# musevlt/origin

Hardware: AMD Instinct MI355X
Metric: voxels/s through DCT+PCA+GLR (ORIGIN hot path) (higher is better)
Workload: dtype f32+f16x2; 1 GPU; synthetic 3681x600x600 cube, Dico_FWHM_2_12 (20 profiles), PSF 25x25, 100x100 areas, dct_order 10, pfa 0.01, Noise_population 50, itermax 100; masked_border=0, glr_spectral_arithmetic=f16x2, tiles=1

## Files before the change

### origin_amd/csrc/common.h

```cpp
#pragma once
#include <hip/hip_runtime.h>

#include <algorithm>
#include <cstdarg>
#include <cstdio>
#include <cstring>
#include <mutex>
#include <vector>

#include "../../include/origin_hip.h"

enum OriginKernelId {
  K_DCT_FIT = 0,
  K_DCT_SUMS,
  K_DCT_STANDARDIZE,
  K_DCT_CONTINUUM,
  K_O2,
  K_PCA_SELECT,
  K_PCA_BMEAN,
  K_PCA_GATHER,
  K_PCA_PROJECT,
  K_PCA_GRAM,
  K_PCA_EIG,
  K_PCA_UVEC,
  K_PCA_DEFLATE_DOT,
  K_PCA_DEFLATE_UPDATE,
  K_PCA_FLUSH,
  K_GLR_SPATIAL,
  K_GLR_SPECTRAL,
  K_GLR_BORDER,
  K_GLR_TABLES,
  K_LOCAL_MAX,
  K_SMALL,
  K_PCA_TOTAL,
  K_LINES_GATHER,
  K_LINES_UVEC,
  K_LINES_PROJECT,
  K_LINES_LS,
  K_LINES_SELECT,
  K_MERGE_BIN,
  K_MERGE_COMP,
  K_MERGE_STAGE1,
  K_MERGE_RENUMBER,
  K_MERGE_STAGE2,
  K_STATS,
  K_COUNT
};

struct OriginProfEvent {
  hipEvent_t a, b;
  int id;
};

constexpr int ORIGIN_TIMER_SLOTS = 64;

struct GrowBuffer {
  void *p = nullptr;
  size_t bytes = 0;
};

struct ForkStream {
  hipStream_t stream = nullptr;
  hipEvent_t fork = nullptr, join = nullptr;
  bool pending = false;
};

struct AllocCache;

struct origin_ctx {
  int device = 0;
  hipStream_t stream = nullptr;
  hipEvent_t ev_start[ORIGIN_TIMER_SLOTS] = {};
  hipEvent_t ev_stop[ORIGIN_TIMER_SLOTS] = {};
  bool ev_made[ORIGIN_TIMER_SLOTS] = {};
  GrowBuffer scratch;
  int num_cu = 0;
  double *ctab = nullptr;
  int ctab_nz = 0, ctab_order = 0;
  int prof_level = 0;
  std::vector<OriginProfEvent> prof_pending;
  std::vector<hipEvent_t> prof_free;
  double prof_ms[K_COUNT] = {};
  long prof_n[K_COUNT] = {};
  void *pca_ws = nullptr;
  void (*pca_ws_free)(void *) = nullptr;
  ForkStream aux;
  GrowBuffer aux_scratch;
  ForkStream side;
  char *stage_buf[2] = {nullptr, nullptr};
  hipEvent_t stage_ev[2] = {nullptr, nullptr};
  bool stage_ready = false;
  void (*pca_tail_hook)(void *user, int n_active, const int *areas) = nullptr;
  void *pca_tail_user = nullptr;
  int pca_tail_max = 0;
  AllocCache *alloc_cache = nullptr;
};

int origin_make_aux_stream(origin_ctx *ctx, hipStream_t *out);
int origin_make_side_stream(origin_ctx *ctx, hipStream_t *out);
int origin_fork_begin(origin_ctx *ctx, ForkStream &f, int (*create)(origin_ctx *, hipStream_t *));
int origin_fork_end(ForkStream &f);
int origin_fork_join(origin_ctx *ctx, ForkStream &f);
int origin_fork_wait(ForkStream &f);

int origin_prof_begin(origin_ctx *ctx, int id);
void origin_prof_end(origin_ctx *ctx, int entry);

struct ProfScope {
  origin_ctx *ctx;
  int entry;
  ProfScope(origin_ctx *c, int id, int level = 1) : ctx(c), entry(-1) {
    if (ctx->prof_level >= level) entry = origin_prof_begin(ctx, id);
  }
  void next(int id) {
    if (entry >= 0) {
      origin_prof_end(ctx, entry);
      entry = origin_prof_begin(ctx, id);
    }
  }
  ~ProfScope() {
    if (entry >= 0) origin_prof_end(ctx, entry);
  }
};

void origin_set_error(const char *fmt, ...);
int origin_grow(GrowBuffer &b, size_t bytes, hipStream_t sync, void **out);
static inline int origin_scratch(origin_ctx *ctx, size_t bytes, void **out) {
  return origin_grow(ctx->scratch, bytes, ctx->stream, out);
}

int origin_spatial_mfma_ok(int Ny, int Nx, int P);
int origin_spatial_mfma_launch(origin_ctx *ctx, int terms, const float *A, const float *W,
                               const float *taps, int Nz, int Ny, int Nx, int P, int accf,
                               float *out, int ry0 = 0, int nry = 0, int rx0 = 0, int nrx = 0);
long origin_spatial_mfma_count(int terms, int Nz, int Ny, int Nx, int P);

struct DevMem {
  origin_ctx *ctx;
  void *p = nullptr;
  explicit DevMem(origin_ctx *c) : ctx(c) {}
  int alloc(size_t bytes) { return origin_malloc(ctx, std::max(bytes, (size_t)256), &p); }
  ~DevMem() {
    if (p) (void)origin_free(ctx, p);
  }
};

struct Carver {
  size_t off = 0;
  char *base = nullptr;
  template <class T>
  T *take(size_t n) {
    T *r = base ? (T *)(base + off) : nullptr;
    off += (n * sizeof(T) + 255) & ~(size_t)255;
    return r;
  }
};

template <class Layout>
int carve_block(origin_ctx *ctx, DevMem &mem, Layout &&layout) {
  Carver c;
  layout(c);
  const int rc = mem.alloc(c.off);
  if (rc) return rc;
  c.off = 0, c.base = (char *)mem.p;
  layout(c);
  return ORIGIN_OK;
}

constexpr long IO_CHUNK_BYTES = 64l << 20;

struct IoStage {
  void *h[2] = {nullptr, nullptr};
  hipEvent_t ev[2] = {nullptr, nullptr};
  ~IoStage() {
    for (int i = 0; i < 2; ++i) {
      if (h[i]) (void)hipHostFree(h[i]);
      if (ev[i]) (void)hipEventDestroy(ev[i]);
    }
  }
};

template <class T>
int put(origin_ctx *ctx, T *d, const std::vector<T> &h) {
  return origin_h2d(ctx, d, h.data(), h.size() * sizeof(T));
}

#define ORIGIN_CHECK_ARG(cond, ...)       \
  do {                                    \
    if (!(cond)) {                        \
      origin_set_error(__VA_ARGS__);      \
      return ORIGIN_E_ARG;                \
    }                                     \
  } while (0)

#define ORIGIN_HIP(call)                                                              \
// ... 42 lines not shown
```

### origin_amd/csrc/ctx.hip

```cpp
#include <sys/mman.h>

#include <algorithm>
#include <cstdlib>
#include <map>
#include <unordered_map>

#include <functional>

#include <cstring>
#include "common.h"

void origin_host_pool_run(int n, const std::function<void(int)> &task);

static thread_local char g_err[1024] = "";

struct AllocCache {
  std::mutex mu;
  std::unordered_map<void *, size_t> live;
  std::multimap<size_t, void *> spare;
  size_t spare_bytes = 0, cap_bytes = 0;
};
constexpr size_t ALLOC_MIN = (size_t)1 << 20;

static size_t alloc_cache_spare(AllocCache *c) {
  std::lock_guard<std::mutex> lk(c->mu);
  return c->spare_bytes;
}

static void alloc_cache_release(origin_ctx *ctx, bool destroy) {
  AllocCache *c = ctx->alloc_cache;
  if (!c) return;
  {
    std::lock_guard<std::mutex> lk(c->mu);
    if (!c->spare.empty()) (void)hipStreamSynchronize(ctx->stream);
    for (auto &kv : c->spare) (void)hipFree(kv.second);
    c->spare.clear();
    c->spare_bytes = 0;
  }
  if (destroy) {
    delete c;
    ctx->alloc_cache = nullptr;
  }
}

__global__ __launch_bounds__(256) void copy_box_kernel(char *__restrict__ dst, long dpy, long dpz,
                                                       const char *__restrict__ src, long spy,
                                                       long spz, int ny, long rowbytes, int vec) {
  const int z = blockIdx.z;
  const int y = blockIdx.y;
  const long x = ((long)blockIdx.x * 256 + threadIdx.x) * vec;
  if (y >= ny || x >= rowbytes) return;
  const char *s = src + (long)z * spz + (long)y * spy + x;
  char *d = dst + (long)z * dpz + (long)y * dpy + x;
  if (vec == 16) {
    *reinterpret_cast<uint4 *>(d) = *reinterpret_cast<const uint4 *>(s);
  } else if (vec == 4) {
    *reinterpret_cast<unsigned *>(d) = *reinterpret_cast<const unsigned *>(s);
  } else {
    *d = *s;
  }
}

void origin_set_error(const char *fmt, ...) {
  va_list ap;
  va_start(ap, fmt);
  vsnprintf(g_err, sizeof(g_err), fmt, ap);
  va_end(ap);
}

int origin_grow(GrowBuffer &b, size_t bytes, hipStream_t sync, void **out) {
  if (bytes > b.bytes) {
    if (b.p) {
      if (sync) ORIGIN_HIP(hipStreamSynchronize(sync));
      ORIGIN_HIP(hipFree(b.p));
      b.p = nullptr;
      b.bytes = 0;
    }
    const size_t want = bytes + bytes / 4 + (1 << 20);
    ORIGIN_HIP(hipMalloc(&b.p, want));
    b.bytes = want;
  }
  *out = b.p;
  return ORIGIN_OK;
}

int origin_make_side_stream(origin_ctx *ctx, hipStream_t *out) {
  const char *e = getenv("ORIGIN_GLR_SIDE_RESERVE");
  const int ncu = ctx->num_cu > 0 ? std::min(ctx->num_cu, 256) : 256;
  int reserve = e ? atoi(e) : ncu / 8;
  reserve = std::max(0, std::min(reserve, ncu - 8));
  uint32_t mask[8] = {0, 0, 0, 0, 0, 0, 0, 0};
  for (int i = 0; i < ncu - reserve; ++i) mask[i >> 5] |= 1u << (i & 31);
  if (hipExtStreamCreateWithCUMask(out, 8, mask) != hipSuccess) {
    (void)hipGetLastError();
    return origin_make_aux_stream(ctx, out);
  }
  return ORIGIN_OK;
}

int origin_make_aux_stream(origin_ctx *, hipStream_t *out) {
  int lo = 0, hi = 0;
  ORIGIN_HIP(hipDeviceGetStreamPriorityRange(&lo, &hi));
  ORIGIN_HIP(hipStreamCreateWithPriority(out, hipStreamNonBlocking, lo));
  return ORIGIN_OK;
}

int origin_fork_begin(origin_ctx *ctx, ForkStream &f, int (*create)(origin_ctx *, hipStream_t *)) {
  if (!f.stream) {
    if (int rc = create(ctx, &f.stream)) return rc;
    ORIGIN_HIP(hipEventCreateWithFlags(&f.fork, hipEventDisableTiming));
    ORIGIN_HIP(hipEventCreateWithFlags(&f.join, hipEventDisableTiming));
  }
  ORIGIN_HIP(hipEventRecord(f.fork, ctx->stream));
  ORIGIN_HIP(hipStreamWaitEvent(f.stream, f.fork, 0));
  return ORIGIN_OK;
}

int origin_fork_end(ForkStream &f) {
  ORIGIN_HIP(hipEventRecord(f.join, f.stream));
  f.pending = true;
  return ORIGIN_OK;
}

int origin_fork_join(origin_ctx *ctx, ForkStream &f) {
  if (f.stream && f.pending) {
    ORIGIN_HIP(hipStreamWaitEvent(ctx->stream, f.join, 0));
    f.pending = false;
  }
  return ORIGIN_OK;
}

int origin_fork_wait(ForkStream &f) {
  if (f.stream && f.pending) {
    ORIGIN_HIP(hipStreamSynchronize(f.stream));
    f.pending = false;
  }
  return ORIGIN_OK;
}

static hipEvent_t prof_event(origin_ctx *ctx) {
  if (!ctx->prof_free.empty()) {
    hipEvent_t e = ctx->prof_free.back();
    ctx->prof_free.pop_back();
    return e;
  }
  hipEvent_t e = nullptr;
  (void)hipEventCreate(&e);
  return e;
}

static void prof_drain(origin_ctx *ctx) {
  for (auto &p : ctx->prof_pending) {
    float ms = 0.f;
    if (p.a && p.b && hipEventSynchronize(p.b) == hipSuccess &&
        hipEventElapsedTime(&ms, p.a, p.b) == hipSuccess) {
      ctx->prof_ms[p.id] += ms;
      ctx->prof_n[p.id] += 1;
    }
    if (p.a) ctx->prof_free.push_back(p.a);
    if (p.b) ctx->prof_free.push_back(p.b);
  }
  ctx->prof_pending.clear();
}

int origin_prof_begin(origin_ctx *ctx, int id) {
  OriginProfEvent p;
  p.a = prof_event(ctx);
  p.b = nullptr;
  p.id = id;
  if (p.a) (void)hipEventRecord(p.a, ctx->stream);
  ctx->prof_pending.push_back(p);
  return (int)ctx->prof_pending.size() - 1;
}

void origin_prof_end(origin_ctx *ctx, int entry) {
  if (entry < 0 || entry >= (int)ctx->prof_pending.size()) return;
  OriginProfEvent &p = ctx->prof_pending[entry];
  p.b = prof_event(ctx);
  if (p.b) (void)hipEventRecord(p.b, ctx->stream);
}

static const char *kKernelNames[K_COUNT] = {
    "dct_fit",         "dct_plane_sums",     "dct_standardize", "dct_continuum", "o2",
    "pca_select",      "pca_bmean",          "pca_gather",      "pca_project",   "pca_gram",
    "pca_eig",         "pca_uvec",
    "pca_deflate_dot", "pca_deflate_finish", "pca_flush", "glr_spatial",     "glr_spectral",  "glr_border", "glr_tables",
    "local_max",       "small",              "pca_total",
    "lines_gather",    "lines_uvec",         "lines_project",   "lines_ls",      "lines_select",
    "merge_bin",       "merge_components",   "merge_stage1",    "merge_renumber", "merge_stage2",
    "cube_moments"};

extern "C" {

int origin_prof_enable(origin_ctx *ctx, int on) {
  ORIGIN_USE(ctx);
  prof_drain(ctx);
  ctx->prof_level = on < 0 ? 0 : (on > 2 ? 2 : on);
  return ORIGIN_OK;
}

int origin_prof_reset(origin_ctx *ctx) {
  ORIGIN_USE(ctx);
  prof_drain(ctx);
  memset(ctx->prof_ms, 0, sizeof(ctx->prof_ms));
  memset(ctx->prof_n, 0, sizeof(ctx->prof_n));
  return ORIGIN_OK;
}

int origin_prof_count(void) { return K_COUNT; }

int origin_prof_get(origin_ctx *ctx, int id, const char **name, double *total_ms, long *launches) {
  ORIGIN_USE(ctx);
  ORIGIN_CHECK_ARG(id >= 0 && id < K_COUNT, "kernel id out of range");
  prof_drain(ctx);
  if (name) *name = kKernelNames[id];
  if (total_ms) *total_ms = ctx->prof_ms[id];
  if (launches) *launches = ctx->prof_n[id];
  return ORIGIN_OK;
}

const char *origin_last_error(void) { return g_err; }

int origin_abi_version(void) { return 1; }

int origin_device_count(int *count) {
  ORIGIN_CHECK_ARG(count, "count is null");
  int n = 0;
  hipError_t e = hipGetDeviceCount(&n);
  if (e != hipSuccess) {
    *count = 0;
    origin_set_error("hipGetDeviceCount: %s", hipGetErrorString(e));
    return ORIGIN_E_NODEVICE;
  }
  *count = n;
  return ORIGIN_OK;
}

int origin_ctx_create(int device, origin_ctx **out) {
  ORIGIN_CHECK_ARG(out, "out is null");
  int n = 0;
  if (hipGetDeviceCount(&n) != hipSuccess || n <= 0) {
    origin_set_error("no HIP device visible");
    return ORIGIN_E_NODEVICE;
  }
  ORIGIN_CHECK_ARG(device >= 0 && device < n, "device %d out of range [0,%d)", device, n);
  ORIGIN_HIP(hipSetDevice(device));
  origin_ctx *ctx = new origin_ctx();
  ctx->device = device;
  hipError_t e = hipStreamCreateWithFlags(&ctx->stream, hipStreamNonBlocking);
  if (e != hipSuccess) {
    delete ctx;
    origin_set_error("hipStreamCreate: %s", hipGetErrorString(e));
    return ORIGIN_E_HIP;
  }
  hipDeviceProp_t prop;
  if (hipGetDeviceProperties(&prop, device) == hipSuccess) ctx->num_cu = prop.multiProcessorCount;
  if (ctx->num_cu <= 0) ctx->num_cu = 256;
  ctx->alloc_cache = new AllocCache();
  const char *gb = getenv("ORIGIN_ALLOC_CACHE_GB");
  ctx->alloc_cache->cap_bytes = (size_t)((gb ? atof(gb) : 96.0) * 1e9);
  *out = ctx;
  return ORIGIN_OK;
}

int origin_ctx_destroy(origin_ctx *ctx) {
  if (!ctx) return ORIGIN_OK;
  hipSetDevice(ctx->device);
  hipStreamSynchronize(ctx->stream);
  for (int i = 0; i < ORIGIN_TIMER_SLOTS; ++i)
    if (ctx->ev_made[i]) {
      hipEventDestroy(ctx->ev_start[i]);
      hipEventDestroy(ctx->ev_stop[i]);
    }
  for (ForkStream *f : {&ctx->aux, &ctx->side})
    if (f->stream) {
      hipStreamSynchronize(f->stream);
      hipStreamDestroy(f->stream);
      hipEventDestroy(f->fork);
      hipEventDestroy(f->join);
    }
  if (ctx->stage_ready) {
    for (int b = 0; b < 2; ++b) {
      hipHostFree(ctx->stage_buf[b]);
      hipEventDestroy(ctx->stage_ev[b]);
    }
  }
  alloc_cache_release(ctx, true);
  if (ctx->aux_scratch.p) hipFree(ctx->aux_scratch.p);
  if (ctx->scratch.p) hipFree(ctx->scratch.p);
  if (ctx->ctab) hipFree(ctx->ctab);
  if (ctx->pca_ws && ctx->pca_ws_free) ctx->pca_ws_free(ctx->pca_ws);
  prof_drain(ctx);
  for (hipEvent_t e : ctx->prof_free) hipEventDestroy(e);
  hipStreamDestroy(ctx->stream);
  delete ctx;
  return ORIGIN_OK;
}

int origin_sync(origin_ctx *ctx) {
  ORIGIN_USE(ctx);
  if (int rc = origin_fork_wait(ctx->side)) return rc;
  ORIGIN_HIP(hipStreamSynchronize(ctx->stream));
  return origin_fork_wait(ctx->aux);
}

int origin_aux_join(origin_ctx *ctx) {
  ORIGIN_USE(ctx);
  return origin_fork_join(ctx, ctx->aux);
}

int origin_device_name(origin_ctx *ctx, char *buf, int buflen) {
  ORIGIN_USE(ctx);
  ORIGIN_CHECK_ARG(buf && buflen > 0, "bad buffer");
  hipDeviceProp_t prop;
  ORIGIN_HIP(hipGetDeviceProperties(&prop, ctx->device));
  snprintf(buf, buflen, "%s (%s, %d CUs)", prop.name, prop.gcnArchName, prop.multiProcessorCount);
  return ORIGIN_OK;
}

int origin_mem_info(origin_ctx *ctx, size_t *free_bytes, size_t *total_bytes) {
  ORIGIN_USE(ctx);
  size_t f = 0, t = 0;
  ORIGIN_HIP(hipMemGetInfo(&f, &t));
  if (free_bytes) *free_bytes = f + alloc_cache_spare(ctx->alloc_cache);
  if (total_bytes) *total_bytes = t;
  return ORIGIN_OK;
}

int origin_stream(origin_ctx *ctx, void **stream) {
  ORIGIN_USE(ctx);
  ORIGIN_CHECK_ARG(stream, "stream is null");
  *stream = (void *)ctx->stream;
  return ORIGIN_OK;
}

int origin_malloc(origin_ctx *ctx, size_t bytes, void **d_ptr) {
  ORIGIN_USE(ctx);
  ORIGIN_CHECK_ARG(d_ptr, "d_ptr is null");
  *d_ptr = nullptr;
  if (bytes == 0) bytes = 16;
  AllocCache *c = ctx->alloc_cache;
  if (bytes >= ALLOC_MIN && c->cap_bytes > 0) {
    std::lock_guard<std::mutex> lk(c->mu);
    auto it = c->spare.lower_bound(bytes);
    if (it != c->spare.end() && it->first - bytes <= bytes / 8) {
      *d_ptr = it->second;
      c->live[it->second] = it->first;
      c->spare_bytes -= it->first;
      c->spare.erase(it);
      return ORIGIN_OK;
    }
  }
  hipError_t e = hipMalloc(d_ptr, bytes);
  if (e == hipErrorOutOfMemory && alloc_cache_spare(c) > 0) {
    (void)hipGetLastError();
    alloc_cache_release(ctx, false);
    e = hipMalloc(d_ptr, bytes);
  }
  if (e != hipSuccess) {
    origin_set_error("hipMalloc of %zu bytes failed: %s", bytes, hipGetErrorString(e));
    return e == hipErrorOutOfMemory ? ORIGIN_E_NOMEM : ORIGIN_E_HIP;
  }
  if (bytes >= ALLOC_MIN && c->cap_bytes > 0) {
    std::lock_guard<std::mutex> lk(c->mu);
    c->live[*d_ptr] = bytes;
  }
  return ORIGIN_OK;
}

int origin_free(origin_ctx *ctx, void *d_ptr) {
  ORIGIN_USE(ctx);
  if (!d_ptr) return ORIGIN_OK;
  AllocCache *c = ctx->alloc_cache;
  {
    std::unique_lock<std::mutex> lk(c->mu);
    auto it = c->live.find(d_ptr);
    if (it != c->live.end()) {
      const size_t sz = it->second;
      c->live.erase(it);
      if (c->spare_bytes + sz <= c->cap_bytes) {
        lk.unlock();
        if (int rc = origin_fork_join(ctx, ctx->aux)) return rc;
        if (int rc = origin_fork_join(ctx, ctx->side)) return rc;
        lk.lock();
// ... 242 lines not shown
```

### origin_amd/csrc/pca.hip

```cpp
#include <algorithm>
#include <cstdlib>
#include <cstring>
#include <chrono>
#include <vector>

#include "common.h"
#include "pca_eig.h"

namespace {

enum {
  DF_AREA = 0, DF_LIST0, DF_N, DF_NB, DF_LD, DF_XP, DF_C, DF_G, DF_Q, DF_NS, DF_CBASE,
  DF_T,
  DF_CN,
  DF_FBOLD,
  DF_LDOLD,
  DF_NOLD,
  DF_SVALID,
  DF_COUNT
};
constexpr int PCA_CAP = 64;
#define DSC(f, k) (D[(long)(f) * nw + (k)])

struct BlockScan {
// ... 760 lines not shown
#pragma unroll 4
  for (int z = z0; z < z1; ++z) acc = fma(uk[z], (double)F[(long)z * S + col], acc);
  if (live) cpart[(long)blockIdx.y * ntot + DSC(DF_CBASE, k) + li] = acc;
}

__global__ __launch_bounds__(256) void deflate_dot_rows_kernel(
    const float *__restrict__ F, int Nz, long S, const int *__restrict__ area_of,
    const int *__restrict__ pos_of, const int *__restrict__ kidx, const long *__restrict__ D,
    int nw, const double *__restrict__ u, int zper, double *__restrict__ cpart, long ntot) {
  const long s = (long)blockIdx.x * 256 + threadIdx.x;
  int k = -1;
  if (s < S) {
    const int a = area_of[s];
    if (a >= 0) k = kidx[a];
  }
  if (!__any(k >= 0)) return;
  const long sc = k >= 0 ? s : (long)blockIdx.x * 256;
  const double *uk = u + (long)(k >= 0 ? k : 0) * Nz;
  const int z0 = blockIdx.y * zper, z1 = min(Nz, z0 + zper);
  double acc = 0.0;
#pragma unroll 4
  for (int z = z0; z < z1; ++z) acc = fma(uk[z], (double)F[(long)z * S + sc], acc);
  if (k >= 0)
    cpart[(long)blockIdx.y * ntot + DSC(DF_CBASE, k) + (pos_of[s] - DSC(DF_LIST0, k))] = acc;
}

__global__ __launch_bounds__(256) void invert_lists_kernel(const int *__restrict__ spx,
                                                           const long *__restrict__ spx_off,
                                                           int *__restrict__ area_of,
                                                           int *__restrict__ pos_of) {
  const int a = blockIdx.y;
  const long o0 = spx_off[a];
  const long i = o0 + (long)blockIdx.x * 256 + threadIdx.x;
  if (i >= spx_off[a + 1]) return;
  const int s = spx[i];
  area_of[s] = a;
  pos_of[s] = (int)i;
}

__global__ __launch_bounds__(256) void deflate_finish_kernel(const int *__restrict__ spx,
                                                             const long *__restrict__ D, int nw,
                                                             int nzs, int Nz, long cb_tot,
                                                             const double *__restrict__ cpart,
                                                             const double *__restrict__ wq,
                                                             double *__restrict__ C, long ntot,
                                                             double *__restrict__ test) {
  const int k = blockIdx.y;
  const int ns = (int)DSC(DF_NS, k);
  const int li = blockIdx.x * 256 + threadIdx.x;
  if (li >= ns) return;
  const int T = (int)DSC(DF_T, k);
  const long pos = DSC(DF_LIST0, k) + li;
  const long ci = DSC(DF_CBASE, k) + li;
  double c = 0.0;
  {
    int q = 0;
    for (; q + 8 <= nzs; q += 8) {
      double v[8];
#pragma unroll
      for (int e = 0; e < 8; ++e) v[e] = cpart[(long)(q + e) * cb_tot + ci];
#pragma unroll
      for (int e = 0; e < 8; ++e) c += v[e];
    }
    for (; q < nzs; ++q) c += cpart[(long)q * cb_tot + ci];
  }
  const double *w = wq + (long)k * PCA_CAP;
  {
    int q = 0;
    for (; q + 8 <= T; q += 8) {
      double v[8];
#pragma unroll
      for (int e = 0; e < 8; ++e) v[e] = C[(long)(q + e) * ntot + pos];
#pragma unroll
      for (int e = 0; e < 8; ++e) c = fma(-w[q + e], v[e], c);
    }
    for (; q < T; ++q) c = fma(-w[q], C[(long)q * ntot + pos], c);
  }
  C[(long)T * ntot + pos] = c;
  const long sp = spx[pos];
  test[sp] = test[sp] - c * c / (double)Nz;
}

constexpr int FLUSH_ZB = 32;
__global__ __launch_bounds__(256, 4) void flush_kernel(const float *X, float *F, int Nz, long S,
                                                    const int *__restrict__ spx,
                                                    const long *__restrict__ FD, int nf,
                                                    const double *__restrict__ U,
                                                    const double *__restrict__ C, long ntot,
                                                    int nxb, int nzb, int out_nx, long out_py,
                                                    long out_pz) {
  __shared__ double Us[FLUSH_ZB][PCA_CAP];
  const long id = blockIdx.x;
  const int low = (int)(id & 7);
  const long rest = id >> 3;
  const int k = (int)(rest % nf);
  const long cz = (rest / nf) * 8 + low;
  if (cz >= (long)nxb * nzb) return;
  const int bx = (int)(cz % nxb), by = (int)(cz / nxb);
  const int ns = (int)FD[(long)2 * nf + k], T = (int)FD[(long)3 * nf + k];
  const int li = bx * 256 + threadIdx.x;
  if (bx * 256 >= ns) return;
  const bool live = li < ns;
  const long pos = FD[(long)1 * nf + k] + (live ? li : ns - 1);
  const long col = spx[pos];
  const long fcol = out_nx > 0 ? (col / out_nx) * out_py + (col % out_nx) : col;
  const long fS = out_nx > 0 ? out_pz : S;
  const double *Ua = U + FD[k] * (long)Nz * PCA_CAP;
  const int z0 = by * FLUSH_ZB;
  for (int i = threadIdx.x; i < FLUSH_ZB * PCA_CAP; i += 256) {
    const int r = i / PCA_CAP, q = i - r * PCA_CAP;
    Us[r][q] = (z0 + r < Nz && q < T) ? Ua[(long)(z0 + r) * PCA_CAP + q] : 0.0;
  }
  __syncthreads();
  double acc[FLUSH_ZB];
#pragma unroll
  for (int r = 0; r < FLUSH_ZB; ++r) acc[r] = 0.0;
  for (int q0 = 0; q0 < T; q0 += 8) {
    double c[8];
#pragma unroll
    for (int e = 0; e < 8; ++e) c[e] = q0 + e < T ? C[(long)(q0 + e) * ntot + pos] : 0.0;
#pragma unroll
    for (int r = 0; r < FLUSH_ZB; r += 2) {
#pragma unroll
      for (int e = 0; e < 8; ++e) {
        acc[r] = fma(Us[r][q0 + e], c[e], acc[r]);
        acc[r + 1] = fma(Us[r + 1][q0 + e], c[e], acc[r + 1]);
      }
      __builtin_amdgcn_sched_barrier(0);
    }
  }
  float xv[FLUSH_ZB];
#pragma unroll
  for (int r = 0; r < FLUSH_ZB; ++r) xv[r] = X[(long)min(z0 + r, Nz - 1) * S + col];
  if (live) {
#pragma unroll
    for (int r = 0; r < FLUSH_ZB; ++r) {
      const int z = z0 + r;
      if (z < Nz) F[(long)z * fS + fcol] = (float)((double)xv[r] - acc[r]);
    }
  }
}

struct DevBuf {
  void *p = nullptr;
  size_t bytes = 0;
  int reserve(origin_ctx *ctx, size_t want) {
    if (want <= bytes) return ORIGIN_OK;
    if (p) {
      ORIGIN_HIP(hipStreamSynchronize(ctx->stream));
      ORIGIN_HIP(hipFree(p));
      p = nullptr;
      bytes = 0;
    }
    const size_t n = want + want / 4 + 4096;
    ORIGIN_HIP(hipMalloc(&p, n));
    bytes = n;
    return ORIGIN_OK;
  }
  void release() {
    if (p) (void)hipFree(p);
    p = nullptr;
    bytes = 0;
  }
  ~DevBuf() { release(); }
};

struct HostBuf {
  void *p = nullptr;
  size_t bytes = 0;
  unsigned flags = 0;
  int reserve(size_t want, unsigned fl) {
    if (want <= bytes && fl == flags) return ORIGIN_OK;
    if (p) (void)hipHostFree(p);
    p = nullptr;
    bytes = 0;
    const size_t n = want + want / 2 + 256;
    ORIGIN_HIP(hipHostMalloc(&p, n, fl));
    bytes = n;
    flags = fl;
    return ORIGIN_OK;
  }
  ~HostBuf() {
    if (p) (void)hipHostFree(p);
  }
};

struct PcaWorkspace {
  DevBuf state, lists, test, desc, xp, g, cv, bu, part, cpart, info, U, C, small, fd;
  DevBuf fb[2];
  DevBuf bgsum;
  DevBuf invert;
  DevBuf work;
  HostBuf h_nnb, h_stage;
};

int gram_launch(origin_ctx *ctx, const double *d_Xp, const long *d_xp_off, const long *d_ld, int Nz,
                int ntiles, const int *d_ti, const int *d_tj, const int *d_ta, long g_total,
                double *d_G, const long *d_g_off, bool skip_reduce = false,
                const double **slab_out = nullptr, int *ksplit_out = nullptr,
                const long *d_n = nullptr) {
  const int ksplit = pca_gram_ksplit(ctx->num_cu, ntiles, Nz);
  void *scr = nullptr;
  int rc = origin_scratch(ctx, (size_t)ksplit * g_total * sizeof(double), &scr);
  if (rc) return rc;
  ProfScope ps(ctx, K_PCA_GRAM, 2);
  hipLaunchKernelGGL(gram_kernel, dim3(ntiles, ksplit), dim3(64), 0, ctx->stream, d_Xp, d_xp_off,
                     d_ld, d_ti, d_tj, d_ta, Nz, ksplit, (double *)scr, d_g_off, g_total, d_n);
  if (slab_out) *slab_out = (const double *)scr;
  if (ksplit_out) *ksplit_out = ksplit;
  if (!skip_reduce)
    hipLaunchKernelGGL(gram_reduce_kernel, dim3(ntiles), dim3(256), 0, ctx->stream,
                       (const double *)scr, g_total, ksplit, d_ld, d_ti, d_tj, d_ta, d_G, d_g_off,
                       d_n);
  ORIGIN_LAUNCH_CHECK();
  return ORIGIN_OK;
}

struct PcaWork {
  int nw = 0;
  long xp = 0, c = 0, g = 0, q = 0;
  long cb = 0;
  int ldmax = 0, nsmax = 0, ntiles = 0;
};

struct PcaRun {
  origin_ctx *ctx;
  PcaWorkspace &W;
  hipStream_t st;
  const float *d_X;
  float *d_F;
  int Nz;
  long S;
  int na;
  const int *d_spx;
  const long *h_spx_off;
  double noise_pop;
  int itermax;
  int *d_mapO2;
  int out_nx;
  long out_py, out_pz;
  const int nsmax_all;
  const bool sel_resident;

  long ntot;
  const float *src;
  float *d_work = nullptr;
  bool debug;
  double *d_thr;
  long *d_spx_off;
  int *d_active, *d_nbiter, *d_n, *d_nb, *d_nstop;
  unsigned *d_selcnt;
  int *d_nuis, *d_bg, *d_bg_pos, *d_npos[2];
  double *d_ssum;
  int *d_dlist, *d_ndiff;
  uint8_t *d_inb;
  int *d_area_of, *d_pos_of;
  double *d_test;
  double *d_U, *d_C;
  int *h_nnb;
  int *d_hostout;
  int iters = 0;
  int gen = 1;
  std::vector<int> counts;
  std::vector<int> T;
  std::vector<long> fb_off, fb_ld, fb_n;
  std::vector<char> s_valid;
  std::vector<char> flushed;
  std::vector<long> D;
  bool tail_fired = false;
  int tail_run = 0, tail_n0 = 0;

  int ns_of(int a) const { return (int)(h_spx_off[a + 1] - h_spx_off[a]); }
  int setup(const double *d_test0, const double *h_thr);
  int flush(bool final, bool only_done = false);
  int select();
  int active_areas(bool *full) const;
  int maybe_fire_tail_hook(int nw, bool full);
  int build_work_list(int nw, PcaWork &w, long *h_trace, int trace_cap);
  int enqueue_chain(const PcaWork &w);
  int report_debug(int nw, const double *d_info);
  void advance(const PcaWork &w);
};

int PcaRun::setup(const double *d_test0, const double *h_thr) {
  int rc;
  const size_t st_bytes = (size_t)na * (sizeof(double) + 4 * sizeof(int)) + sizeof(int) * 2 +
                          (size_t)(na + 1) * sizeof(long) + 64;
  if ((rc = W.state.reserve(ctx, st_bytes))) return rc;
  d_thr = (double *)W.state.p;
  d_spx_off = (long *)(d_thr + na);
  d_active = (int *)(d_spx_off + na + 1);
  d_nbiter = d_active + na;
  d_n = d_nbiter + na;
  d_nb = d_n + na;
  d_nstop = d_nb + na;
  d_selcnt = (unsigned *)(d_nstop + 1);
  std::vector<int> ones(na, 1);
  ORIGIN_HIP(hipMemcpyAsync(d_thr, h_thr, (size_t)na * sizeof(double), hipMemcpyHostToDevice, st));
  ORIGIN_HIP(hipMemcpyAsync(d_spx_off, h_spx_off, (size_t)(na + 1) * sizeof(long),
                            hipMemcpyHostToDevice, st));
  ORIGIN_HIP(hipMemcpyAsync(d_active, ones.data(), (size_t)na * sizeof(int), hipMemcpyHostToDevice,
                            st));
  ORIGIN_HIP(hipMemsetAsync(d_nbiter, 0, (size_t)na * sizeof(int), st));
  ORIGIN_HIP(hipMemsetAsync(d_nstop, 0, 2 * sizeof(int), st));
  ORIGIN_HIP(hipStreamSynchronize(st));
  if ((rc = W.lists.reserve(ctx, (size_t)5 * ntot * sizeof(int)))) return rc;
  d_nuis = (int *)W.lists.p;
  d_bg = d_nuis + ntot;
  d_bg_pos = d_bg + ntot;
  d_npos[0] = d_bg_pos + ntot;
  d_npos[1] = d_npos[0] + ntot;
  fb_off.assign(na, -1);
  fb_ld.assign(na, 0);
  fb_n.assign(na, 0);
  if ((rc = W.bgsum.reserve(ctx, (size_t)na * Nz * sizeof(double) +
                                     (size_t)(ntot + na) * sizeof(int) + (size_t)ntot)))
    return rc;
  d_ssum = (double *)W.bgsum.p;
  d_dlist = (int *)(d_ssum + (size_t)na * Nz);
  d_ndiff = d_dlist + ntot;
  d_inb = (uint8_t *)(d_ndiff + na);
  ORIGIN_HIP(hipMemsetAsync(d_inb, 0, (size_t)ntot, st));
  s_valid.assign(na, 0);
  if ((rc = W.invert.reserve(ctx, (size_t)2 * S * sizeof(int)))) return rc;
  d_area_of = (int *)W.invert.p;
  d_pos_of = d_area_of + S;
  ORIGIN_HIP(hipMemsetAsync(d_area_of, 0xFF, (size_t)S * sizeof(int), st));
  if (nsmax_all > 0)
    hipLaunchKernelGGL(invert_lists_kernel, dim3(cdiv(nsmax_all, 256), na), dim3(256), 0, st, d_spx,
                       d_spx_off, d_area_of, d_pos_of);
  if ((rc = W.test.reserve(ctx, (size_t)S * sizeof(double)))) return rc;
  d_test = (double *)W.test.p;
  ORIGIN_HIP(hipMemcpyAsync(d_test, d_test0, (size_t)S * sizeof(double), hipMemcpyDeviceToDevice,
                            st));
  if ((rc = W.U.reserve(ctx, (size_t)na * Nz * PCA_CAP * sizeof(double)))) return rc;
  if ((rc = W.C.reserve(ctx, (size_t)PCA_CAP * ntot * sizeof(double)))) return rc;
  d_U = (double *)W.U.p, d_C = (double *)W.C.p;
  T.assign(na, 0);
  flushed.assign(na, 0);
  counts.assign(2 * (size_t)na, 0);

  if ((rc = W.h_nnb.reserve((size_t)(2 * na + 1) * sizeof(int),
                            hipHostMallocMapped | hipHostMallocCoherent)))
    return rc;
  h_nnb = (int *)W.h_nnb.p;
  memset(h_nnb, 0, (size_t)(2 * na + 1) * sizeof(int));
  ORIGIN_HIP(hipHostGetDevicePointer((void **)&d_hostout, h_nnb, 0));
  return ORIGIN_OK;
}

int PcaRun::flush(bool final, bool only_done) {
  const bool strided = out_nx > 0;
  float *dst = d_F;
  if (strided && !final) {
    int rw = W.work.reserve(ctx, (size_t)Nz * S * sizeof(float));
    if (rw) return rw;
    if (!d_work && ntot < S)
      ORIGIN_HIP(hipMemcpyAsync(W.work.p, d_X, (size_t)Nz * S * sizeof(float),
                                hipMemcpyDeviceToDevice, st));
    d_work = (float *)W.work.p;
    dst = d_work;
  }
  const bool to_strided = strided && final;
  const bool all = src != dst;
  std::vector<int> areas;
  for (int a = 0; a < na; ++a) {
    if (flushed[a] || (only_done && counts[a] >= 2)) continue;
    if ((all || T[a] > 0) && ns_of(a) > 0) areas.push_back(a);
  }
  const int nf = (int)areas.size();
  if (nf > 0) {
    std::vector<long> fd((size_t)4 * nf);
    int nsmax = 0;
    for (int k = 0; k < nf; ++k) {
      const int a = areas[k];
      fd[k] = a;
      fd[(size_t)nf + k] = h_spx_off[a];
      fd[(size_t)2 * nf + k] = ns_of(a);
      fd[(size_t)3 * nf + k] = T[a];
      nsmax = std::max(nsmax, ns_of(a));
    }
    int r;
    if ((r = W.fd.reserve(ctx, fd.size() * sizeof(long)))) return r;
    ORIGIN_HIP(hipMemcpyAsync(W.fd.p, fd.data(), fd.size() * sizeof(long), hipMemcpyHostToDevice,
                              st));
    ORIGIN_HIP(hipStreamSynchronize(st));
    ProfScope ps(ctx, K_PCA_FLUSH, 2);
    const int nxb = cdiv(nsmax, 256), nzb = cdiv(Nz, FLUSH_ZB);
    const long ngroups = ((long)nxb * nzb + 7) / 8;
    hipLaunchKernelGGL(flush_kernel, dim3((unsigned)(ngroups * nf * 8)), dim3(256), 0, st, src, dst,
                       Nz, S, d_spx, (const long *)W.fd.p, nf, d_U, d_C, ntot, nxb, nzb,
                       to_strided ? out_nx : 0, out_py, out_pz);
    ORIGIN_LAUNCH_CHECK();
  }
  if (only_done) {
    for (int a = 0; a < na; ++a)
      if (counts[a] < 2) flushed[a] = 1, T[a] = 0;
    return ORIGIN_OK;
  }
  for (int a = 0; a < na; ++a) T[a] = 0;
  std::fill(fb_off.begin(), fb_off.end(), -1L);
  std::fill(s_valid.begin(), s_valid.end(), (char)0);
  src = dst;
  return ORIGIN_OK;
}

int PcaRun::select() {
  {
    ProfScope ps(ctx, K_PCA_SELECT, 2);
    const SelectArgs sel{d_spx, d_spx_off, d_test, d_thr, noise_pop, itermax, d_active, d_nbiter,
                         d_nstop, d_mapO2, d_nuis, d_bg, d_npos[iters & 1], d_bg_pos, d_n, d_nb,
                         d_inb, d_dlist, d_ndiff, d_hostout, d_selcnt, gen};
    if (sel_resident)
      hipLaunchKernelGGL(pca_select_fast_kernel, dim3(na), dim3(1024),
                         (size_t)nsmax_all * sizeof(int), st, sel);
    else
      hipLaunchKernelGGL(pca_select_kernel, dim3(na), dim3(1024), 0, st, sel);
  }
  ORIGIN_LAUNCH_CHECK();
  int *flag = h_nnb + 2 * na;
  const auto t_start = std::chrono::steady_clock::now();
  long polls = 0;
  while (__atomic_load_n(flag, __ATOMIC_ACQUIRE) != gen) {
    __builtin_ia32_pause();
    if ((++polls & 0xfffff) == 0 &&
        std::chrono::steady_clock::now() - t_start > std::chrono::seconds(5)) {
      ORIGIN_HIP(hipStreamSynchronize(st));
      if (__atomic_load_n(flag, __ATOMIC_ACQUIRE) != gen) {
        origin_set_error("greedy PCA: the selection kernel did not report back");
        return ORIGIN_E_HIP;
      }
    }
  }
  ++gen;
  memcpy(counts.data(), h_nnb, 2 * (size_t)na * sizeof(int));
  return ORIGIN_OK;
}

int PcaRun::active_areas(bool *full) const {
  int nw = 0;
  *full = false;
  for (int a = 0; a < na; ++a)
    if (counts[a] >= 2) {
      ++nw;
      *full = *full || T[a] >= PCA_CAP;
    }
  return nw;
}

int PcaRun::maybe_fire_tail_hook(int nw, bool full) {
  int n_active_sum = 0;
  for (int a = 0; a < na; ++a)
    if (counts[a] >= 2) n_active_sum += counts[a];
  if (nw <= ctx->pca_tail_max && iters >= 1) {
    if (tail_run++ == 0) tail_n0 = n_active_sum;
  } else {
    tail_run = 0;
  }
  if (!ctx->pca_tail_hook || tail_fired || tail_run < 3 ||
      10 * (long)n_active_sum < 6 * (long)tail_n0 || d_work || full)
    return ORIGIN_OK;
  tail_fired = true;
  int rc = flush(true, true);
  if (rc) return rc;
  std::vector<int> act;
  for (int a = 0; a < na; ++a)
    if (counts[a] >= 2) act.push_back(a);
  ctx->pca_tail_hook(ctx->pca_tail_user, (int)act.size(), act.data());
  return ORIGIN_OK;
}

int PcaRun::build_work_list(int nw, PcaWork &w, long *h_trace, int trace_cap) {
  w = PcaWork();
  w.nw = nw;
  D.assign((size_t)DF_COUNT * nw, 0);
  std::vector<int> ti, tj, ta;
  std::vector<int> kidx(na, -1);
  int k = 0;
  long nsum = 0;
  for (int a = 0; a < na; ++a) {
    const int n = counts[a];
    if (n < 2) continue;
    const int ld = (n + 15) / 16 * 16;
    const int ns = ns_of(a);
    D[(size_t)DF_AREA * nw + k] = a;
    D[(size_t)DF_LIST0 * nw + k] = h_spx_off[a];
    D[(size_t)DF_N * nw + k] = n;
    D[(size_t)DF_NB * nw + k] = counts[na + a];
    D[(size_t)DF_LD * nw + k] = ld;
    D[(size_t)DF_XP * nw + k] = w.xp;
    D[(size_t)DF_C * nw + k] = w.c;
    D[(size_t)DF_G * nw + k] = w.g;
    D[(size_t)DF_Q * nw + k] = w.q;
    D[(size_t)DF_NS * nw + k] = ns;
    D[(size_t)DF_CBASE * nw + k] = w.cb;
    D[(size_t)DF_T * nw + k] = T[a];
    const bool have = fb_off[a] >= 0 && T[a] >= 1;
    D[(size_t)DF_FBOLD * nw + k] = have ? fb_off[a] : -1;
    D[(size_t)DF_LDOLD * nw + k] = fb_ld[a];
    D[(size_t)DF_NOLD * nw + k] = fb_n[a];
    D[(size_t)DF_SVALID * nw + k] = sel_resident && s_valid[a];
    s_valid[a] = sel_resident;
    w.xp += (long)Nz * ld;
    w.c += ld;
    w.g += (long)ld * ld;
    w.q += (long)EIG_QROWS * ld;
    w.cb += ns;
    w.ldmax = std::max(w.ldmax, ld);
    w.nsmax = std::max(w.nsmax, ns);
    nsum += n;
    const int Tt = (ld + 31) / 32;
    for (int i = 0; i < Tt; ++i)
      for (int j = i; j < Tt; ++j) ti.push_back(i), tj.push_back(j), ta.push_back(k);
    kidx[a] = k;
    ++k;
  }
  const int ntiles = w.ntiles = (int)ti.size();
  if (h_trace && iters < trace_cap) {
    h_trace[2 * iters] = nw;
    h_trace[2 * iters + 1] = nsum;
  }
  const size_t dbytes = D.size() * sizeof(long), tbytes = (size_t)3 * ntiles * sizeof(int);
  const size_t kbytes = (size_t)na * sizeof(int);
  int rc;
  if ((rc = W.desc.reserve(ctx, dbytes + tbytes + kbytes))) return rc;
  if (dbytes + tbytes + kbytes > W.h_stage.bytes &&
      (rc = W.h_stage.reserve((dbytes + tbytes + kbytes) * 2, hipHostMallocDefault)))
    return rc;
  char *h_stage = (char *)W.h_stage.p;
  memcpy(h_stage, D.data(), dbytes);
  int *ht = (int *)(h_stage + dbytes);
  memcpy(ht, ti.data(), (size_t)ntiles * sizeof(int));
  memcpy(ht + ntiles, tj.data(), (size_t)ntiles * sizeof(int));
  memcpy(ht + 2 * (size_t)ntiles, ta.data(), (size_t)ntiles * sizeof(int));
  memcpy(ht + 3 * (size_t)ntiles, kidx.data(), kbytes);
  ORIGIN_HIP(hipMemcpyAsync(W.desc.p, h_stage, dbytes + tbytes + kbytes, hipMemcpyHostToDevice, st));
  return ORIGIN_OK;
}

int PcaRun::enqueue_chain(const PcaWork &w) {
  int rc;
  const int nw = w.nw, ntiles = w.ntiles;
  const size_t dbytes = D.size() * sizeof(long);
  const long *dD = (const long *)W.desc.p;
  const int *d_ti = (const int *)((char *)W.desc.p + dbytes), *d_tj = d_ti + ntiles,
            *d_ta = d_tj + ntiles, *d_kidx = d_ta + ntiles;
  const long *dLD = dD + (size_t)DF_LD * nw, *dXP = dD + (size_t)DF_XP * nw;
// ... 147 lines not shown
}

}

extern "C" {

int origin_pca_gram(origin_ctx *ctx, const double *d_Xp, const long *d_xp_off, const long *d_ld,
                    int Nz, int ntiles, const int *d_tile_i, const int *d_tile_j,
                    const int *d_tile_a, long g_total, double *d_G, const long *d_g_off) {
  ORIGIN_USE(ctx);
  ORIGIN_CHECK_ARG(d_Xp && d_xp_off && d_ld && d_tile_i && d_tile_j && d_tile_a && d_G &&
                       d_g_off && Nz > 0 && ntiles > 0 && g_total > 0,
                   "bad arguments");
  return gram_launch(ctx, d_Xp, d_xp_off, d_ld, Nz, ntiles, d_tile_i, d_tile_j, d_tile_a, g_total,
                     d_G, d_g_off);
}

int origin_pca_set_tail_hook(origin_ctx *ctx, void (*hook)(void *, int, const int *), void *user,
                             int max_active) {
  ORIGIN_CHECK_ARG(ctx && max_active >= 0, "bad argument");
  ctx->pca_tail_hook = hook;
  ctx->pca_tail_user = user;
  ctx->pca_tail_max = max_active;
  return ORIGIN_OK;
}

int origin_pca_run_into(origin_ctx *ctx, const float *d_X, float *d_F, int Nz, long S, int na,
                        const int *d_spx, const long *h_spx_off, const double *d_test0,
                        const double *h_thr, double noise_pop, int itermax, int *d_mapO2,
                        int *h_nstop, int *h_iters, long *h_trace, int trace_cap, int out_nx,
                        long out_py, long out_pz) {
  ORIGIN_USE(ctx);
  const bool strided = out_nx > 0;
  ORIGIN_CHECK_ARG(!strided || (d_X && d_X != d_F && S % out_nx == 0 && out_py >= out_nx &&
                                out_pz >= (S / out_nx) * out_py),
                   "strided output needs a separate contiguous input and consistent pitches");
  ORIGIN_CHECK_ARG(d_F && d_spx && h_spx_off && d_test0 && h_thr && d_mapO2 && h_nstop &&
                       Nz > 0 && S > 0 && na > 0,
                   "bad arguments");
  ORIGIN_CHECK_ARG(noise_pop > 0 && itermax >= 0, "bad Noise_population / itermax");
  ProfScope ps_total(ctx, K_PCA_TOTAL, 1);
  if (!d_X) d_X = d_F;
  const long ntot = h_spx_off[na];
  ORIGIN_CHECK_ARG(ntot >= 0 && ntot <= S, "area lists longer than the field");
  hipStream_t st = ctx->stream;
  if (h_iters) *h_iters = 0;
  *h_nstop = 0;
  ORIGIN_HIP(hipMemsetAsync(d_mapO2, 0, (size_t)S * sizeof(int), st));
  if (d_X != d_F && ntot < S) {
    if (strided) {
      int rcb = origin_copy_box(ctx, 2, d_F, out_py, out_pz, d_X, out_nx, S, Nz, (int)(S / out_nx),
                                out_nx, (int)sizeof(float));
      if (rcb) return rcb;
    } else {
      ORIGIN_HIP(hipMemcpyAsync(d_F, d_X, (size_t)Nz * S * sizeof(float), hipMemcpyDeviceToDevice, st));
    }
  }
  if (ntot == 0) return ORIGIN_OK;

  if (!ctx->pca_ws) {
    ctx->pca_ws = new PcaWorkspace();
    ctx->pca_ws_free = [](void *p) { delete (PcaWorkspace *)p; };
  }
  int nsmax_all = 0;
  for (int a = 0; a < na; ++a)
    nsmax_all = std::max(nsmax_all, (int)(h_spx_off[a + 1] - h_spx_off[a]));
  PcaRun R{ctx, *(PcaWorkspace *)ctx->pca_ws, st, d_X, d_F, Nz, S, na, d_spx, h_spx_off,
           noise_pop, itermax, d_mapO2, out_nx, out_py, out_pz, nsmax_all,
           nsmax_all <= 1024 * SEL_EPT};
  R.ntot = ntot;
  R.src = d_X;
  R.debug = getenv("ORIGIN_PCA_DEBUG") != nullptr;
  int rc;
  if ((rc = R.setup(d_test0, h_thr))) return rc;

  double t_build = 0, t_enq = 0;
  using Clock = std::chrono::steady_clock;
  for (;;) {
    const auto tp0 = Clock::now();
    if ((rc = R.select())) return rc;
    bool full;
    const int nw = R.active_areas(&full);
    if (nw == 0) break;
    if ((rc = R.maybe_fire_tail_hook(nw, full))) return rc;
    if (full && (rc = R.flush(false))) return rc;
    PcaWork work;
    if ((rc = R.build_work_list(nw, work, h_trace, trace_cap))) return rc;
    const auto tp1 = Clock::now();
    if ((rc = R.enqueue_chain(work))) return rc;
    R.advance(work);
    t_build += std::chrono::duration<double>(tp1 - tp0).count();
    t_enq += std::chrono::duration<double>(Clock::now() - tp1).count();
  }
  if (getenv("ORIGIN_PCA_TIMING"))
    fprintf(stderr, "[pca] host loop: %d iterations, build %.2f ms, enqueue %.2f ms\n", R.iters,
            1e3 * t_build, 1e3 * t_enq);
  if ((rc = R.flush(true))) return rc;
  ORIGIN_HIP(hipMemcpyAsync(R.h_nnb, R.d_nstop, sizeof(int), hipMemcpyDeviceToHost, st));
  ORIGIN_HIP(hipStreamSynchronize(st));
  *h_nstop = R.h_nnb[0];
  if (h_iters) *h_iters = R.iters;
  return ORIGIN_OK;
}

int origin_pca_run(origin_ctx *ctx, const float *d_X, float *d_F, int Nz, long S, int na,
                   const int *d_spx, const long *h_spx_off, const double *d_test0,
                   const double *h_thr, double noise_pop, int itermax, int *d_mapO2, int *h_nstop,
                   int *h_iters, long *h_trace, int trace_cap) {
  return origin_pca_run_into(ctx, d_X, d_F, Nz, S, na, d_spx, h_spx_off, d_test0, h_thr, noise_pop,
                             itermax, d_mapO2, h_nstop, h_iters, h_trace, trace_cap, 0, 0, 0);
}

}
```

Measured before the change: 27.17 billion voxels/s.

## Flush finished PCA areas early on a CU-masked side stream

Adds a separate flush stream that is CU-masked to reserve part of the device. When only a few areas remain active, areas that have already converged are flushed on that stream so their work overlaps the tail iterations of the remaining PCA loop. The flush descriptors are passed by value as kernel arguments instead of through a host-to-device copy. The aim is to shorten the serial tail of the PCA loop. The cost is extra fork/join synchronisation and contention for CUs with the main stream.

```diff
diff --git a/origin_amd/csrc/common.h b/origin_amd/csrc/common.h
--- a/origin_amd/csrc/common.h
+++ b/origin_amd/csrc/common.h
@@ -50,6 +50,7 @@
 struct OriginProfEvent {
   hipEvent_t a, b;
   int id;
+  hipStream_t stream;
 };
 
 constexpr int ORIGIN_TIMER_SLOTS = 64;
@@ -87,6 +88,7 @@
   ForkStream aux;
   GrowBuffer aux_scratch;
   ForkStream side;
+  ForkStream flush;
   char *stage_buf[2] = {nullptr, nullptr};
   hipEvent_t stage_ev[2] = {nullptr, nullptr};
   bool stage_ready = false;
@@ -98,19 +100,20 @@
 
 int origin_make_aux_stream(origin_ctx *ctx, hipStream_t *out);
 int origin_make_side_stream(origin_ctx *ctx, hipStream_t *out);
+int origin_make_flush_stream(origin_ctx *ctx, hipStream_t *out);
 int origin_fork_begin(origin_ctx *ctx, ForkStream &f, int (*create)(origin_ctx *, hipStream_t *));
 int origin_fork_end(ForkStream &f);
 int origin_fork_join(origin_ctx *ctx, ForkStream &f);
 int origin_fork_wait(ForkStream &f);
 
-int origin_prof_begin(origin_ctx *ctx, int id);
+int origin_prof_begin(origin_ctx *ctx, int id, hipStream_t st = nullptr);
 void origin_prof_end(origin_ctx *ctx, int entry);
 
 struct ProfScope {
   origin_ctx *ctx;
   int entry;
-  ProfScope(origin_ctx *c, int id, int level = 1) : ctx(c), entry(-1) {
-    if (ctx->prof_level >= level) entry = origin_prof_begin(ctx, id);
+  ProfScope(origin_ctx *c, int id, int level = 1, hipStream_t st = nullptr) : ctx(c), entry(-1) {
+    if (ctx->prof_level >= level) entry = origin_prof_begin(ctx, id, st);
   }
   void next(int id) {
     if (entry >= 0) {
diff --git a/origin_amd/csrc/ctx.hip b/origin_amd/csrc/ctx.hip
--- a/origin_amd/csrc/ctx.hip
+++ b/origin_amd/csrc/ctx.hip
@@ -84,10 +84,8 @@
   return ORIGIN_OK;
 }
 
-int origin_make_side_stream(origin_ctx *ctx, hipStream_t *out) {
-  const char *e = getenv("ORIGIN_GLR_SIDE_RESERVE");
+static int make_masked_stream(origin_ctx *ctx, int reserve, hipStream_t *out) {
   const int ncu = ctx->num_cu > 0 ? std::min(ctx->num_cu, 256) : 256;
-  int reserve = e ? atoi(e) : ncu / 8;
   reserve = std::max(0, std::min(reserve, ncu - 8));
   uint32_t mask[8] = {0, 0, 0, 0, 0, 0, 0, 0};
   for (int i = 0; i < ncu - reserve; ++i) mask[i >> 5] |= 1u << (i & 31);
@@ -96,6 +94,17 @@
     return origin_make_aux_stream(ctx, out);
   }
   return ORIGIN_OK;
+}
+
+int origin_make_side_stream(origin_ctx *ctx, hipStream_t *out) {
+  const char *e = getenv("ORIGIN_GLR_SIDE_RESERVE");
+  const int ncu = ctx->num_cu > 0 ? std::min(ctx->num_cu, 256) : 256;
+  return make_masked_stream(ctx, e ? atoi(e) : ncu / 8, out);
+}
+
+constexpr int PCA_FLUSH_RESERVE = 32;
+int origin_make_flush_stream(origin_ctx *ctx, hipStream_t *out) {
+  return make_masked_stream(ctx, PCA_FLUSH_RESERVE, out);
 }
 
 int origin_make_aux_stream(origin_ctx *, hipStream_t *out) {
@@ -163,12 +172,13 @@
   ctx->prof_pending.clear();
 }
 
-int origin_prof_begin(origin_ctx *ctx, int id) {
+int origin_prof_begin(origin_ctx *ctx, int id, hipStream_t st) {
   OriginProfEvent p;
   p.a = prof_event(ctx);
   p.b = nullptr;
   p.id = id;
-  if (p.a) (void)hipEventRecord(p.a, ctx->stream);
+  p.stream = st ? st : ctx->stream;
+  if (p.a) (void)hipEventRecord(p.a, p.stream);
   ctx->prof_pending.push_back(p);
   return (int)ctx->prof_pending.size() - 1;
 }
@@ -177,7 +187,7 @@
   if (entry < 0 || entry >= (int)ctx->prof_pending.size()) return;
   OriginProfEvent &p = ctx->prof_pending[entry];
   p.b = prof_event(ctx);
-  if (p.b) (void)hipEventRecord(p.b, ctx->stream);
+  if (p.b) (void)hipEventRecord(p.b, p.stream);
 }
 
 static const char *kKernelNames[K_COUNT] = {
@@ -272,7 +282,7 @@
       hipEventDestroy(ctx->ev_start[i]);
       hipEventDestroy(ctx->ev_stop[i]);
     }
-  for (ForkStream *f : {&ctx->aux, &ctx->side})
+  for (ForkStream *f : {&ctx->aux, &ctx->side, &ctx->flush})
     if (f->stream) {
       hipStreamSynchronize(f->stream);
       hipStreamDestroy(f->stream);
@@ -300,6 +310,7 @@
 int origin_sync(origin_ctx *ctx) {
   ORIGIN_USE(ctx);
   if (int rc = origin_fork_wait(ctx->side)) return rc;
+  if (int rc = origin_fork_wait(ctx->flush)) return rc;
   ORIGIN_HIP(hipStreamSynchronize(ctx->stream));
   return origin_fork_wait(ctx->aux);
 }
diff --git a/origin_amd/csrc/pca.hip b/origin_amd/csrc/pca.hip
--- a/origin_amd/csrc/pca.hip
+++ b/origin_amd/csrc/pca.hip
@@ -866,13 +866,22 @@
 }
 
 constexpr int FLUSH_ZB = 32;
-__global__ __launch_bounds__(256, 4) void flush_kernel(const float *X, float *F, int Nz, long S,
-                                                    const int *__restrict__ spx,
-                                                    const long *__restrict__ FD, int nf,
-                                                    const double *__restrict__ U,
-                                                    const double *__restrict__ C, long ntot,
-                                                    int nxb, int nzb, int out_nx, long out_py,
-                                                    long out_pz) {
+constexpr int FLUSH_BY_VALUE = 64;
+struct FlushDescMem {
+  const long *__restrict__ p;
+  __device__ __forceinline__ long at(int f, int nf, int k) const { return p[(long)f * nf + k]; }
+};
+struct FlushDescArg {
+  long v[4][FLUSH_BY_VALUE];
+  __device__ __forceinline__ long at(int f, int, int k) const { return v[f][k]; }
+};
+
+template <class Desc>
+__device__ __forceinline__ void flush_body(const float *X, float *F, int Nz, long S,
+                                           const int *__restrict__ spx, const Desc &FD, int nf,
+                                           const double *__restrict__ U,
+                                           const double *__restrict__ C, long ntot, int nxb,
+                                           int nzb, int out_nx, long out_py, long out_pz) {
   __shared__ double Us[FLUSH_ZB][PCA_CAP];
   const long id = blockIdx.x;
   const int low = (int)(id & 7);
@@ -881,15 +890,15 @@
   const long cz = (rest / nf) * 8 + low;
   if (cz >= (long)nxb * nzb) return;
   const int bx = (int)(cz % nxb), by = (int)(cz / nxb);
-  const int ns = (int)FD[(long)2 * nf + k], T = (int)FD[(long)3 * nf + k];
+  const int ns = (int)FD.at(2, nf, k), T = (int)FD.at(3, nf, k);
   const int li = bx * 256 + threadIdx.x;
   if (bx * 256 >= ns) return;
   const bool live = li < ns;
-  const long pos = FD[(long)1 * nf + k] + (live ? li : ns - 1);
+  const long pos = FD.at(1, nf, k) + (live ? li : ns - 1);
   const long col = spx[pos];
   const long fcol = out_nx > 0 ? (col / out_nx) * out_py + (col % out_nx) : col;
   const long fS = out_nx > 0 ? out_pz : S;
-  const double *Ua = U + FD[k] * (long)Nz * PCA_CAP;
+  const double *Ua = U + FD.at(0, nf, k) * (long)Nz * PCA_CAP;
   const int z0 = by * FLUSH_ZB;
   for (int i = threadIdx.x; i < FLUSH_ZB * PCA_CAP; i += 256) {
     const int r = i / PCA_CAP, q = i - r * PCA_CAP;
@@ -923,6 +932,23 @@
       if (z < Nz) F[(long)z * fS + fcol] = (float)((double)xv[r] - acc[r]);
     }
   }
+}
+
+__global__ __launch_bounds__(256, 4) void flush_kernel(const float *X, float *F, int Nz, long S,
+                                                    const int *__restrict__ spx,
+                                                    const long *__restrict__ FD, int nf,
+                                                    const double *__restrict__ U,
+                                                    const double *__restrict__ C, long ntot,
+                                                    int nxb, int nzb, int out_nx, long out_py,
+                                                    long out_pz) {
+  flush_body(X, F, Nz, S, spx, FlushDescMem{FD}, nf, U, C, ntot, nxb, nzb, out_nx, out_py, out_pz);
+}
+
+__global__ __launch_bounds__(256, 4) void flush_early_kernel(
+    const float *X, float *F, int Nz, long S, const int *__restrict__ spx, const FlushDescArg FD,
+    int nf, const double *__restrict__ U, const double *__restrict__ C, long ntot, int nxb, int nzb,
+    int out_nx, long out_py, long out_pz) {
+  flush_body(X, F, Nz, S, spx, FD, nf, U, C, ntot, nxb, nzb, out_nx, out_py, out_pz);
 }
 
 struct DevBuf {
@@ -1056,7 +1082,8 @@
 
   int ns_of(int a) const { return (int)(h_spx_off[a + 1] - h_spx_off[a]); }
   int setup(const double *d_test0, const double *h_thr);
-  int flush(bool final, bool only_done = false);
+  int flush(bool final);
+  int flush_done_early(bool full);
   int select();
   int active_areas(bool *full) const;
   int maybe_fire_tail_hook(int nw, bool full);
@@ -1064,6 +1091,7 @@
   int enqueue_chain(const PcaWork &w);
   int report_debug(int nw, const double *d_info);
   void advance(const PcaWork &w);
+  ~PcaRun() { (void)origin_fork_wait(ctx->flush); }
 };
 
 int PcaRun::setup(const double *d_test0, const double *h_thr) {
@@ -1133,7 +1161,9 @@
   return ORIGIN_OK;
 }
 
-int PcaRun::flush(bool final, bool only_done) {
+int PcaRun::flush(bool final) {
+  int r;
+  if ((r = origin_fork_join(ctx, ctx->flush))) return r;
   const bool strided = out_nx > 0;
   float *dst = d_F;
   if (strided && !final) {
@@ -1148,10 +1178,8 @@
   const bool to_strided = strided && final;
   const bool all = src != dst;
   std::vector<int> areas;
-  for (int a = 0; a < na; ++a) {
-    if (flushed[a] || (only_done && counts[a] >= 2)) continue;
-    if ((all || T[a] > 0) && ns_of(a) > 0) areas.push_back(a);
-  }
+  for (int a = 0; a < na; ++a)
+    if (!flushed[a] && (all || T[a] > 0) && ns_of(a) > 0) areas.push_back(a);
   const int nf = (int)areas.size();
   if (nf > 0) {
     std::vector<long> fd((size_t)4 * nf);
@@ -1164,7 +1192,6 @@
       fd[(size_t)3 * nf + k] = T[a];
       nsmax = std::max(nsmax, ns_of(a));
     }
-    int r;
     if ((r = W.fd.reserve(ctx, fd.size() * sizeof(long)))) return r;
     ORIGIN_HIP(hipMemcpyAsync(W.fd.p, fd.data(), fd.size() * sizeof(long), hipMemcpyHostToDevice,
                               st));
@@ -1177,16 +1204,52 @@
                        to_strided ? out_nx : 0, out_py, out_pz);
     ORIGIN_LAUNCH_CHECK();
   }
-  if (only_done) {
-    for (int a = 0; a < na; ++a)
-      if (counts[a] < 2) flushed[a] = 1, T[a] = 0;
-    return ORIGIN_OK;
-  }
   for (int a = 0; a < na; ++a) T[a] = 0;
   std::fill(fb_off.begin(), fb_off.end(), -1L);
   std::fill(s_valid.begin(), s_valid.end(), (char)0);
   src = dst;
   return ORIGIN_OK;
+}
+
+constexpr int EARLY_FLUSH_ACTIVE = 3;
+int PcaRun::flush_done_early(bool full) {
+  if (d_work || full) return ORIGIN_OK;
+  const bool all = src != d_F;
+  std::vector<int> areas;
+  for (int a = 0; a < na; ++a) {
+    if (flushed[a] || counts[a] >= 2) continue;
+    if ((all || T[a] > 0) && ns_of(a) > 0) areas.push_back(a);
+  }
+  int rc = ORIGIN_OK;
+  if (!areas.empty()) {
+    if ((rc = origin_fork_begin(ctx, ctx->flush, origin_make_flush_stream))) return rc;
+    hipStream_t fs = ctx->flush.stream;
+    ProfScope ps(ctx, K_PCA_FLUSH, 2, fs);
+    const int nzb = cdiv(Nz, FLUSH_ZB);
+    for (size_t k0 = 0; k0 < areas.size(); k0 += FLUSH_BY_VALUE) {
+      const int nf = (int)std::min(areas.size() - k0, (size_t)FLUSH_BY_VALUE);
+      FlushDescArg fd = {};
+      int nsmax = 0;
+      for (int k = 0; k < nf; ++k) {
+        const int a = areas[k0 + k];
+        fd.v[0][k] = a;
+        fd.v[1][k] = h_spx_off[a];
+        fd.v[2][k] = ns_of(a);
+        fd.v[3][k] = T[a];
+        nsmax = std::max(nsmax, ns_of(a));
+      }
+      const int nxb = cdiv(nsmax, 256);
+      const long ngroups = ((long)nxb * nzb + 7) / 8;
+      hipLaunchKernelGGL(flush_early_kernel, dim3((unsigned)(ngroups * nf * 8)), dim3(256), 0, fs,
+                         src, d_F, Nz, S, d_spx, fd, nf, d_U, d_C, ntot, nxb, nzb, out_nx, out_py,
+                         out_pz);
+    }
+    ORIGIN_LAUNCH_CHECK();
+  }
+  for (int a = 0; a < na; ++a)
+    if (counts[a] < 2) flushed[a] = 1, T[a] = 0;
+  if (!areas.empty()) rc = origin_fork_end(ctx->flush);
+  return rc;
 }
 
 int PcaRun::select() {
@@ -1245,8 +1308,8 @@
       10 * (long)n_active_sum < 6 * (long)tail_n0 || d_work || full)
     return ORIGIN_OK;
   tail_fired = true;
-  int rc = flush(true, true);
-  if (rc) return rc;
+  int rc = flush_done_early(full);
+  if (rc || (rc = origin_fork_join(ctx, ctx->flush))) return rc;
   std::vector<int> act;
   for (int a = 0; a < na; ++a)
     if (counts[a] >= 2) act.push_back(a);
@@ -1560,6 +1623,7 @@
     bool full;
     const int nw = R.active_areas(&full);
     if (nw == 0) break;
+    if (nw <= EARLY_FLUSH_ACTIVE && (rc = R.flush_done_early(full))) return rc;
     if ((rc = R.maybe_fire_tail_hook(nw, full))) return rc;
     if (full && (rc = R.flush(false))) return rc;
     PcaWork work;
```

New measurement: 26.96 billion voxels/s. Within noise of the previous version (-0.8%).
